# bupt-ai-cz/HIAST

Measured on AMD Instinct MI355X. Metric: self-training images/sec (fwd+bwd+pseudo-label) at 1024x512, higher is better.
Workload: dtype fp16

## Files before the change

### hiast_amd/_lib.py

```python
import ctypes
import os

import torch

_HERE = os.path.dirname(os.path.abspath(__file__))
LIB_PATH = os.environ.get("HIAST_LIB") or os.path.join(_HERE, "csrc", "libhiast_hip.so")

c_int, c_i64, c_f32, c_sz, c_vp = (ctypes.c_int, ctypes.c_int64, ctypes.c_float, ctypes.c_size_t,
                                   ctypes.c_void_p)

SIGNATURES = {
    "hiast_version": (c_int, []),
    "hiast_error_string": (ctypes.c_char_p, [c_int]),
    "hiast_upsample_bilinear_ac_fwd": (c_int, [c_vp, c_vp] + [c_int] * 6 + [c_vp]),
    "hiast_upsample_bilinear_ac_bwd": (c_int, [c_vp, c_vp] + [c_int] * 6 + [c_vp]),
    "hiast_plabel_pass1_workspace_bytes": (c_sz, [c_int]),
    "hiast_plabel_pass1": (c_int, [c_vp] + [c_int] * 6 + [c_vp, c_vp, c_vp, c_vp, c_sz, c_vp]),
    "hiast_plabel_pass2": (c_int, [c_vp, c_vp, c_vp, c_int, c_int, c_i64, c_vp, c_vp, c_vp, c_vp]),
    "hiast_plabel_strided_hist_workspace_bytes": (c_sz, [c_i64, c_int]),
    "hiast_plabel_strided_hist": (c_int, [c_vp, c_vp, c_i64, c_int, c_int, c_vp, c_vp, c_vp, c_vp, c_sz, c_vp]),
    "hiast_tta_fused": (c_int, [c_vp] * 6 + [c_int] * 5 + [c_vp, c_vp, c_vp]),
    "hiast_dinput_fwd": (c_int, [c_vp, c_int, c_vp] + [c_int] * 6 + [c_vp]),
    "hiast_dinput_bwd": (c_int, [c_vp, c_int, c_vp, c_vp, c_vp] + [c_int] * 6 + [c_vp]),
    "hiast_st_loss_workspace_bytes": (c_sz, [c_int] * 6),
    "hiast_st_loss_fwd": (c_int, [c_vp, c_vp, c_vp] + [c_int] * 8 + [c_vp, c_vp, c_sz, c_vp]),
    "hiast_st_loss_bwd": (c_int, [c_vp, c_vp, c_vp] + [c_int] * 8 + [c_vp, c_vp, c_vp, c_vp, c_sz, c_vp]),
    "hiast_aspp_wpack_bytes": (c_sz, [c_int, c_int]),
    "hiast_aspp_workspace_bytes": (c_sz, [c_int] * 5),
    "hiast_aspp_pack_weights": (c_int, [c_vp] * 8 + [c_int, c_int, c_vp, c_vp]),
    "hiast_aspp_fwd": (c_int, [c_vp, c_vp, c_vp] + [c_int] * 5 + [c_vp, c_vp, c_sz, c_vp]),
    "hiast_aspp_bwd_data": (c_int, [c_vp, c_vp, c_vp] + [c_int] * 5 + [c_vp, c_vp]),
    "hiast_aspp_bwd_weight": (c_int, [c_vp] * 7 + [c_int] * 5 + [c_vp, c_vp, c_sz, c_vp]),
    "hiast_aspp2_np": (c_int, [c_int]),
    "hiast_aspp2_workspace_bytes": (c_sz, [c_int] * 6),
    "hiast_aspp2_pack_weights": (c_int, [c_vp] * 8 + [c_int, c_int, c_vp, c_vp, c_vp, c_vp]),
    "hiast_aspp2_fwd": (c_int, [c_vp, c_int, c_vp, c_vp, c_vp] + [c_int] * 5 + [c_vp, c_vp, c_sz, c_vp]),
    "hiast_aspp2_bwd": (c_int, [c_vp] * 9 + [c_int] * 5 + [c_vp, c_int, c_vp, c_sz, c_vp]),
    "hiast_bn_workspace_bytes": (c_sz, [c_int, c_int]),
    "hiast_bn_stats": (c_int, [c_vp, c_int, c_int, c_i64, c_int, c_vp, c_vp]),
    "hiast_bn_act_apply": (c_int, [c_vp] * 8 + [c_int, ctypes.c_double, c_f32, c_f32, c_int, c_vp, c_vp,
                                   c_int, c_int, c_i64, c_int, c_vp]),
    "hiast_bn_act_bwd_stats": (c_int, [c_vp] * 5 + [c_int, c_int, c_int, c_i64, c_int, c_vp, c_vp]),
    "hiast_bn_act_bwd_apply": (c_int, [c_vp] * 7 + [c_int, ctypes.c_double, c_int, c_vp, c_vp, c_vp, c_vp,
                                       c_int, c_int, c_i64, c_int, c_vp]),
    "hiast_bn_act_nhwc_infer": (c_int, [c_vp] * 6 + [c_f32, c_int, c_i64, c_int, c_int, c_vp]),
    "hiast_igemm_bn_act": (c_int, [c_vp] * 6 + [c_f32, c_vp, c_int, c_vp] + [c_int] * 10 + [c_vp, c_int, c_vp, c_int, c_vp]),
    "hiast_igemm_set_cosched": (c_int, [c_int]),
    "hiast_igemm_set_half": (c_int, [c_int]),
    "hiast_device_cus": (c_int, []),
    "hiast_set_reserve_cus": (c_int, [c_int]),
    "hiast_get_reserve_cus": (c_int, []),
    "hiast_stream_create_reserved": (c_int, [c_vp, c_int]),
    "hiast_stream_destroy": (c_int, [c_vp]),
    "hiast_igemm_stats_rows": (c_int, [c_i64, c_int, c_int, c_int, c_int]),
    "hiast_igemm_dgrad_bn_stats": (c_int, [c_vp, c_vp, c_vp] + [c_int] * 7 + [c_vp] * 6 + [c_int, c_int, c_vp]),
    "hiast_xconv_dgrad_gated_bn_stats_rows": (c_int, [c_i64, c_int, c_int]),
    "hiast_xconv_dgrad_gated_bn_stats": (c_int, [c_vp] * 10 + [c_i64, c_int, c_int, c_int, c_vp]),
    "hiast_igemm_dgrad_s2": (c_int, [c_vp, c_vp, c_vp] + [c_int] * 6 + [c_vp]),
    "hiast_igemm_dgrad_bn_stats_rows": (c_int, [c_i64, c_int, c_int, c_int]),
    "hiast_bn_nhwc_stats_from_partial": (c_int, [c_vp, c_int, c_int, c_vp, c_vp]),
    "hiast_conv_wgrad_workspace_bytes": (c_sz, [c_int] * 6),
    "hiast_conv_wgrad_nhwc": (c_int, [c_vp, c_vp, c_vp] + [c_int] * 9 + [c_vp, c_sz, c_vp]),
    "hiast_conv_wgrad_group_workspace_bytes": (c_sz, [c_vp, c_int]),
    "hiast_conv_wgrad_group_nhwc": (c_int, [c_vp, c_int, c_int, c_vp, c_sz, c_vp]),
    "hiast_conv_wgrad_small_workspace_bytes": (c_sz, [c_int] * 6),
    "hiast_conv_wgrad_small_nhwc": (c_int, [c_vp, c_vp, c_vp] + [c_int] * 9 + [c_vp, c_sz, c_vp]),
    "hiast_pack_conv_weight": (c_int, [c_vp, c_int, c_int, c_int, c_int, c_int, c_vp, c_vp, c_vp]),
    "hiast_bn_nhwc_workspace_bytes": (c_sz, [c_int]),
    "hiast_bn_nhwc_stats": (c_int, [c_vp, c_i64, c_int, c_vp, c_vp, c_sz, c_int, c_vp]),
    "hiast_bn_nhwc_apply": (c_int, [c_vp] * 8 + [ctypes.c_double, c_f32, c_f32, c_int, c_vp, c_vp, c_i64, c_int, c_vp,
                                    c_int, c_vp]),
    "hiast_bn_nhwc_apply_partial": (c_int, [c_vp] * 8 + [c_int, ctypes.c_double, c_f32, c_f32, c_int, c_vp, c_vp, c_i64,
                                            c_int, c_vp, c_int, c_vp]),
    "hiast_bn_nhwc_bwd_stats": (c_int, [c_vp] * 7 + [c_int, c_i64, c_int, c_vp, c_vp, c_sz, c_int, c_vp]),
    "hiast_bn_nhwc_bwd_apply": (c_int, [c_vp] * 8 + [ctypes.c_double, c_int, c_vp, c_vp, c_vp, c_vp, c_i64, c_int, c_int,
                                        c_vp]),
    "hiast_pack_conv_weight_multi": (c_int, [c_vp, c_vp, c_vp, c_int, c_int, c_vp]),
    "hiast_split_planes": (c_int, [c_vp, c_vp, c_i64, c_int, c_int, c_vp]),
    "hiast_stem_tail": (c_int, [c_vp, c_int, c_vp, c_vp, c_vp, c_vp, c_f32, c_vp, c_int, c_int, c_int, c_int, c_int, c_vp]),
    "hiast_stem_eval": (c_int, [c_vp] * 6 + [c_f32, c_vp, c_int, c_int, c_int, c_int, c_vp]),
    "hiast_stem_train_blocks": (c_int, [c_int] * 3),
    "hiast_stem_train_fwd": (c_int, [c_vp, c_vp, c_vp, c_vp, c_int, c_int, c_int, c_int, c_vp]),
    "hiast_stem_wgrad_workspace_bytes": (c_sz, [c_int] * 3),
    "hiast_stem_wgrad": (c_int, [c_vp, c_vp, c_vp, c_int, c_int, c_int, c_int, c_vp, c_sz, c_vp]),
    "hiast_ema_update": (c_int, [c_vp, c_vp, c_vp, c_int, c_f32, c_f32, c_vp]),
    "hiast_normalize_u8": (c_int, [c_vp, c_vp, c_int, c_i64, c_vp, c_vp, c_vp]),
    "hiast_maxpool3x3s2_nhwc_fwd": (c_int, [c_vp, c_vp, c_vp, c_int, c_int, c_int, c_int, c_int, c_vp]),
    "hiast_maxpool3x3s2_nhwc_bwd": (c_int, [c_vp, c_vp, c_vp, c_int, c_int, c_int, c_int, c_int, c_vp]),
    "hiast_multi_copy": (c_int, [c_vp, c_int, c_vp]),
    "hiast_aug_geometry_u8": (c_int, [c_vp] * 6 + [c_int] * 4 + [c_vp]),
    "hiast_aug_hist_u8": (c_int, [c_vp] * 5 + [c_int, c_i64, c_vp]),
    "hiast_aug_colour_u8": (c_int, [c_vp] * 5 + [c_int, c_i64, c_vp]),
    "hiast_adam_prepare": (c_int, [c_vp, c_vp, c_vp, c_vp]),
    "hiast_adam_step": (c_int, [c_vp, c_vp, c_vp, c_int, ctypes.c_double, ctypes.c_double, c_f32, c_f32, c_vp, c_vp]),
    "hiast_confusion_hist": (c_int, [c_vp, c_vp, c_i64, c_int, c_vp, c_vp, c_vp, c_vp]),
}



class WgradJob(ctypes.Structure):
    _fields_ = [("dy", c_vp), ("x", c_vp), ("dw", c_vp)] + [(n, ctypes.c_int32) for n in
                                                             ("B", "H", "W", "Cin", "Cout", "taps", "stride", "dil")]


NBINS = 15361
PROB_FX_SHIFT = 30
IGNORE = 255

_lib = None


class HiastLibraryError(RuntimeError):
    pass


def load():
    global _lib
    if _lib is not None:
        return _lib
    if not os.path.exists(LIB_PATH):
        raise HiastLibraryError(
            "libhiast_hip.so is not built (%s). Build it with `python -c 'import __graft_entry__ as g; "
            "g.build()'` or `make -C hiast_amd/csrc`; there is no fallback path." % LIB_PATH)
    lib = ctypes.CDLL(LIB_PATH)
    for name, (res, args) in SIGNATURES.items():
        try:
            fn = getattr(lib, name)
        except AttributeError as e:
            raise HiastLibraryError("libhiast_hip.so does not export %s" % name) from e
        fn.restype = res
        fn.argtypes = args
    if lib.hiast_version() != 6:
        raise HiastLibraryError("libhiast_hip.so ABI version mismatch")
    _lib = lib
    return lib


# ... 17 lines not shown
```

### hiast_amd/csrc/igemm.hip

```cpp
#include "igemm_kernel.h"

namespace hiast {

template <int PL>
__device__ __forceinline__ size_t ig_wp_elem(int n, int t, int k, int taps, int KO)
{
    const size_t row = ((size_t)n * taps + t) * PL * KO;
    return PL == 2 ? row + (size_t)(k >> 5) * 64 + (k & 31) : row + k;
}

template <int PL, bool F16 = false>
__global__ __launch_bounds__(256) void pack_conv_weight_kernel(const float* __restrict__ w,
                                                               unsigned short* __restrict__ wp,
                                                               unsigned short* __restrict__ wpt, int N, int K, int taps,
                                                               int mode)
{
    const long long idx = (long long)blockIdx.x * 256 + threadIdx.x;
    if (idx >= (long long)N * taps * K) return;
    const int k = (int)(idx % K);
    const int t = (int)((idx / K) % taps);
    const int n = (int)(idx / ((long long)K * taps));
    const float v = w[((size_t)n * K + k) * taps + t];
    unsigned short h, l = 0;
    if (F16) h = H16<true>::enc(v);
// ... 104 lines not shown
        const int c = (int)((i * 8) - m * C);
        const float4 a = reinterpret_cast<const float4*>(x)[2 * i], b = reinterpret_cast<const float4*>(x)[2 * i + 1];
        const float v[8] = {a.x, a.y, a.z, a.w, b.x, b.y, b.z, b.w};
        unsigned ph[4], pl_[4];
#pragma unroll
        for (int q = 0; q < 4; ++q) {
            unsigned short h0, l0, h1, l1;
            ig_split(v[2 * q], h0, l0);
            ig_split(v[2 * q + 1], h1, l1);
            ph[q] = (unsigned)h0 | ((unsigned)h1 << 16);
            pl_[q] = (unsigned)l0 | ((unsigned)l1 << 16);
        }
        unsigned short* dst = p + ig_elem<2>((size_t)m, c, C);
        *reinterpret_cast<uint4*>(dst) = make_uint4(ph[0], ph[1], ph[2], ph[3]);
        *reinterpret_cast<uint4*>(dst + 32) = make_uint4(pl_[0], pl_[1], pl_[2], pl_[3]);
    }
}

__global__ __launch_bounds__(256) void from_planes_kernel(const unsigned short* __restrict__ p, float* __restrict__ x,
                                                          long long M, int C)
{
    const long long total8 = M * C / 8;
    for (long long i = (long long)blockIdx.x * 256 + threadIdx.x; i < total8; i += (long long)gridDim.x * 256) {
        const long long m = (i * 8) / C;
        const int c = (int)((i * 8) - m * C);
        const unsigned short* src = p + ig_elem<2>((size_t)m, c, C);
        const uint4 h = *reinterpret_cast<const uint4*>(src), l = *reinterpret_cast<const uint4*>(src + 32);
        const unsigned wh[4] = {h.x, h.y, h.z, h.w}, wl[4] = {l.x, l.y, l.z, l.w};
        float v[8];
#pragma unroll
        for (int q = 0; q < 4; ++q) {
            v[2 * q] = __uint_as_float(wh[q] << 16) + __uint_as_float(wl[q] << 16);
            v[2 * q + 1] = __uint_as_float(wh[q] & 0xFFFF0000u) + __uint_as_float(wl[q] & 0xFFFF0000u);
        }
        reinterpret_cast<float4*>(x)[2 * i] = make_float4(v[0], v[1], v[2], v[3]);
        reinterpret_cast<float4*>(x)[2 * i + 1] = make_float4(v[4], v[5], v[6], v[7]);
    }
}

}

const IgEnv& hiast_ig_env()
{
    static const IgEnv env = [] {
        IgEnv e;
        const char* v = getenv("HIAST_IGEMM_HALF");
        e.half = v ? (atoi(v) != 0) : -1;
        v = getenv("HIAST_IGEMM_BN");
        const int bn = v ? atoi(v) : 0;
        e.bn = (bn == 64 || bn == 128 || bn == 256) ? bn : 0;
        e.ragged_off = getenv("HIAST_IGEMM_RAGGED") != nullptr;
        v = getenv("HIAST_IGEMM_COSCHED");
        e.cosched0 = v && atoi(v) != 0;
        return e;
    }();
    return env;
}
static thread_local int ig_cosched_tls = -1, ig_half_tls = -1;
int hiast_ig_cosched_tls_get() { return ig_cosched_tls; }
int hiast_ig_half_tls_get() { return ig_half_tls; }
extern "C" int hiast_igemm_set_half(int v)
{
    const int prev = ig_half_tls;
    ig_half_tls = v < 0 ? -1 : (v != 0);
    return prev;
}
extern "C" int hiast_igemm_set_cosched(int on)
{
    const int prev = ig_cosched_tls;
    ig_cosched_tls = on < 0 ? -1 : (on != 0);
    return prev;
}

int hiast_xconv_ok(int64_t M, int K, int N, int planes, int taps, int out_f32, int has_bn, int has_res, int relu,
                   int has_gate, int gate_mask, int has_stats);
int hiast_xconv_stats_rows(int64_t M, int N);
int hiast_xconv_launch(const void* x, const void* wp, const float* gamma, const float* beta, const float* mean,
                       const float* var, float eps, const void* res, int relu, void* y, int64_t M, int K, int N,
                       float* stats, const void* res_gate, int f16, hipStream_t st);
int hiast_xconv2_ok(int64_t M, int K, int N, int planes, int taps, int out_f32, int has_bn, int has_res, int relu,
                    int has_gate, int has_stats);
int hiast_xconv2_launch(const void* x, const void* wp, const float* gamma, const float* beta, const float* mean,
                        const float* var, float eps, const void* res, int relu, void* y, int64_t M, int N, hipStream_t st);
int hiast_igemm_launch_f16(const void* x, const void* wp, const float* gamma, const float* beta, const float* mean,
                           const float* var, float eps, const void* res, int relu, void* y, int64_t M, int K, int N, int taps,
                           hiast::IGeo geo, float* stats, const void* res_gate, int gate_mask, hipStream_t st, int stats_mode,
                           int out_f32, int stats_rows);

static int igemm_launch_mode(const void* x, const void* wp, const float* gamma, const float* beta, const float* mean,
                             const float* var, float eps, const void* res, int relu, void* y, int64_t M, int K, int N,
                             int taps, int H, int W, int stride, int dil, int fmt, int out_f32, hipStream_t st,
                             float* stats, const void* res_gate, int gate_mask, int stats_mode, int stats_rows)
{
    if (!hiast_fmt_ok(fmt)) return HIAST_E_RANGE;
    const int planes = hiast_fmt_planes(fmt), f16 = fmt == HIAST_FMT_FP16;
    if (stats_mode == 2) {
        if (!stats || !res || !mean || !var || planes != 1 || out_f32 || relu || res_gate || N % 8) return HIAST_E_RANGE;
    } else {
        if (stats && (planes != 1 || out_f32 || res || relu)) return HIAST_E_RANGE;
        if ((stats || res_gate) && mean) return HIAST_E_RANGE;
    }
    if (res_gate && (planes != 1 || !res || relu || out_f32 || (!gate_mask && (((uintptr_t)res_gate) & 15)))) return HIAST_E_RANGE;
    if (!x || !wp || !y || (mean && !var)) return HIAST_E_ARG;
    if (M <= 0 || K <= 0 || N <= 0) return HIAST_E_ARG;
    if ((planes != 1 && planes != 2) || (taps != 1 && taps != 9)) return HIAST_E_RANGE;
    if ((K * planes) % 64 != 0 || N % 64 != 0 || M > (1ll << 31) - 512) return HIAST_E_RANGE;
    if (out_f32 && res) return HIAST_E_RANGE;
    if ((((uintptr_t)x) | ((uintptr_t)wp) | ((uintptr_t)y) | ((uintptr_t)res)) & 15) return HIAST_E_RANGE;
    hiast::IGeo geo = {0, 0, 0, 0, 1, 1};
    size_t in_pix = (size_t)M;
    if (taps != 1 && stride == -2) {
        if (H <= 0 || W <= 0 || dil != 1 || planes != 1 || out_f32) return HIAST_E_ARG;
        const int Hs = (H - 1) / 2 + 1, Ws = (W - 1) / 2 + 1;
        if (M % ((int64_t)H * W) != 0) return HIAST_E_ARG;
        geo = {Hs, Ws, H, W, -2, 1};
        in_pix = (size_t)(M / ((int64_t)H * W)) * Hs * Ws;
    } else if (taps != 1) {
        if (H <= 0 || W <= 0 || stride <= 0 || dil <= 0) return HIAST_E_ARG;
        const int Ho = (H - 1) / stride + 1, Wo = (W - 1) / stride + 1;
        if (M % ((int64_t)Ho * Wo) != 0) return HIAST_E_ARG;
        geo = {H, W, Ho, Wo, stride, dil};
        in_pix = (size_t)(M / ((int64_t)Ho * Wo)) * H * W;
    }
    if (in_pix * planes * K * 2 >= (1ull << 31) || (size_t)N * taps * planes * K * 2 >= (1ull << 31)) return HIAST_E_RANGE;
    if (stats_mode != 2 &&
        hiast_xconv_ok(M, K, N, planes, taps, out_f32, mean != nullptr, res != nullptr, relu, res_gate != nullptr, gate_mask,
                       stats != nullptr)) {
        if (stats && stats_rows != hiast_xconv_stats_rows(M, N)) return HIAST_E_ARG;
        return hiast_xconv_launch(x, wp, gamma, beta, mean, var, eps, res, relu, y, M, K, N, stats, res_gate, f16, st);
    }
    if (stats_mode == 0 && !f16 &&
        hiast_xconv2_ok(M, K, N, planes, taps, out_f32, mean != nullptr, res != nullptr, relu, res_gate != nullptr, stats != nullptr))
        return hiast_xconv2_launch(x, wp, gamma, beta, mean, var, eps, res, relu, y, M, N, st);
    if (f16)
        return hiast_igemm_launch_f16(x, wp, gamma, beta, mean, var, eps, res, relu, y, M, K, N, taps, geo, stats, res_gate,
                                      gate_mask, st, stats_mode, out_f32, stats_rows);
    if (planes == 2) {
        if (out_f32) return launch_igemm_t<2, true>(x, wp, gamma, beta, mean, var, eps, res, relu, y, M, K, N, taps, geo, stats, res_gate, gate_mask, st, stats_mode, stats_rows);
        return launch_igemm_t<2, false>(x, wp, gamma, beta, mean, var, eps, res, relu, y, M, K, N, taps, geo, stats, res_gate, gate_mask, st, stats_mode, stats_rows);
    }
    if (out_f32) return launch_igemm_t<1, true>(x, wp, gamma, beta, mean, var, eps, res, relu, y, M, K, N, taps, geo, stats, res_gate, gate_mask, st, stats_mode, stats_rows);
    return launch_igemm_t<1, false>(x, wp, gamma, beta, mean, var, eps, res, relu, y, M, K, N, taps, geo, stats, res_gate, gate_mask, st, stats_mode, stats_rows);
}

int hiast_igemm_launch(const void* x, const void* wp, const float* gamma, const float* beta, const float* mean,
                       const float* var, float eps, const void* res, int relu, void* y, int64_t M, int K, int N,
                       int taps, int H, int W, int stride, int dil, int fmt, int out_f32, hipStream_t st,
                       float* stats, const void* res_gate, int gate_mask, int stats_rows)
{
    return igemm_launch_mode(x, wp, gamma, beta, mean, var, eps, res, relu, y, M, K, N, taps, H, W, stride, dil, fmt,
                             out_f32, st, stats, res_gate, gate_mask, stats ? 1 : 0, stats_rows);
}

extern "C" int hiast_igemm_dgrad_bn_stats(const void* dy, const void* wpt, void* da, int B, int H, int W, int Cin, int Cout,
                                          int taps, int dil, const void* bn_x, const float* gamma, const float* beta,
                                          const float* save_mean, const float* save_invstd, float* partial, int partial_rows,
                                          int fmt, hiast_stream_t stream)
{
    if (fmt != HIAST_FMT_BF16 && fmt != HIAST_FMT_FP16) return HIAST_E_RANGE;
    if (B <= 0 || H <= 0 || W <= 0) return HIAST_E_ARG;
    if (!bn_x || !save_mean || !save_invstd || !partial) return HIAST_E_ARG;
    if ((((uintptr_t)save_mean) | ((uintptr_t)save_invstd) | ((uintptr_t)gamma) | ((uintptr_t)beta)) & 15) return HIAST_E_RANGE;
    return igemm_launch_mode(dy, wpt, gamma, beta, save_mean, save_invstd, 0.0f, bn_x, 0, da, (int64_t)B * H * W, Cin, Cout,
                             taps, H, W, 1, dil, fmt, 0, (hipStream_t)stream, partial, nullptr, 0, 2, partial_rows);
}

extern "C" int hiast_igemm_dgrad_s2(const void* dy, const void* wpt, void* dx, int B, int H, int W, int Cin, int Cout, int fmt,
                                    hiast_stream_t stream)
{
    if (fmt != HIAST_FMT_BF16 && fmt != HIAST_FMT_FP16) return HIAST_E_RANGE;
    if (B <= 0 || H <= 0 || W <= 0) return HIAST_E_ARG;
    return igemm_launch_mode(dy, wpt, nullptr, nullptr, nullptr, nullptr, 0.0f, nullptr, 0, dx, (int64_t)B * H * W, Cout, Cin, 9,
                             H, W, -2, 1, fmt, 0, (hipStream_t)stream, nullptr, nullptr, 0, 0, 0);
}

extern "C" int hiast_igemm_dgrad_bn_stats_rows(int64_t M, int Cin, int Cout, int taps)
{
    if (M <= 0) return 0;
    const int bm = ig_block_rows(M, Cin, Cout, taps, 0);
    return (int)((M + bm - 1) / bm);
}

extern "C" int hiast_igemm_bn_act(const void* x, const void* wp, const float* gamma, const float* beta,
                                  const float* mean, const float* var, float eps, const void* res, int relu, void* y,
                                  int B, int H, int W, int Cin, int Cout, int taps, int stride, int dil, int fmt,
                                  int out_f32, float* stats, int stats_rows, const void* res_gate, int gate_mask,
                                  hiast_stream_t stream)
{
    if (B <= 0 || H <= 0 || W <= 0) return HIAST_E_ARG;
    if (taps == 1 && stride != 1) return HIAST_E_RANGE;
    const int Ho = taps == 1 ? H : (H - 1) / stride + 1, Wo = taps == 1 ? W : (W - 1) / stride + 1;
    return hiast_igemm_launch(x, wp, gamma, beta, mean, var, eps, res, relu, y, (int64_t)B * Ho * Wo, Cin, Cout, taps, H,
                              W, stride, dil, fmt, out_f32, (hipStream_t)stream, stats, res_gate, gate_mask, stats_rows);
}

#ifdef IG_STAMP
namespace hiast {
__global__ void ig_stamp_copy_kernel(unsigned* dst)
{
    for (int i = blockIdx.x * blockDim.x + threadIdx.x; i < 1024 * 8 * 8 + 32 * 64; i += gridDim.x * blockDim.x) dst[i] = ig_stamp_buf[i];
}
}
extern "C" int hiast_igemm_debug_stamps(unsigned* dst_device)
{
    hipLaunchKernelGGL(hiast::ig_stamp_copy_kernel, dim3(64), dim3(256), 0, 0, dst_device);
    return (int)hipDeviceSynchronize();
}
#endif

extern "C" int hiast_igemm_stats_rows(int64_t M, int Cin, int Cout, int taps, int fmt)
{
    const int planes = hiast_fmt_planes(fmt);
    if (M <= 0 || Cin <= 0 || Cout <= 0) return 0;
    if (hiast_xconv_ok(M, Cin, Cout, planes, taps, 0, 0, 0, 0, 0, 0, 1)) return hiast_xconv_stats_rows(M, Cout);
    const int bm = ig_block_rows(M, Cin, Cout, taps, 0);
    return (int)((M + bm - 1) / bm);
}

extern "C" int hiast_pack_conv_weight(const float* w, int N, int K, int taps, int fmt, int transpose, void* wp,
                                      void* wpt, hiast_stream_t stream)
{
    if (!w || !wp) return HIAST_E_ARG;
    if (N <= 0 || K <= 0 || taps <= 0) return HIAST_E_ARG;
    const int planes = fmt;
    if (!hiast_fmt_ok(fmt) || transpose < 0 || transpose > 2) return HIAST_E_RANGE;
    if (transpose == 2 && !wpt) return HIAST_E_ARG;
    const long long total = (long long)N * K * taps;
    if (N % 64 == 0 && K % 64 == 0 && taps <= 9 && !((((uintptr_t)wp) | ((uintptr_t)wpt)) & 15)) {
        const dim3 tg((unsigned)((N / 64) * (K / 64)));
        const size_t lds_bytes = (size_t)32 * taps * hiast::PK_PITCH * sizeof(unsigned short);
        if (planes == HIAST_FMT_SPLIT_BF16)
            hipLaunchKernelGGL(hiast::pack_conv_weight_tiled_kernel<2>, tg, dim3(256), lds_bytes, (hipStream_t)stream, w,
                               (unsigned short*)wp, (unsigned short*)wpt, N, K, taps, transpose);
        else if (planes == HIAST_FMT_FP16)
            hipLaunchKernelGGL((hiast::pack_conv_weight_tiled_kernel<1, true>), tg, dim3(256), lds_bytes, (hipStream_t)stream, w,
                               (unsigned short*)wp, (unsigned short*)wpt, N, K, taps, transpose);
        else
            hipLaunchKernelGGL(hiast::pack_conv_weight_tiled_kernel<1>, tg, dim3(256), lds_bytes, (hipStream_t)stream, w,
                               (unsigned short*)wp, (unsigned short*)wpt, N, K, taps, transpose);
        HIAST_CHECK_LAUNCH();
        return 0;
    }
    const dim3 grid((unsigned)((total + 255) / 256));
    if (planes == HIAST_FMT_SPLIT_BF16)
        hipLaunchKernelGGL(hiast::pack_conv_weight_kernel<2>, grid, dim3(256), 0, (hipStream_t)stream, w,
                           (unsigned short*)wp, (unsigned short*)wpt, N, K, taps, transpose);
    else if (planes == HIAST_FMT_FP16)
        hipLaunchKernelGGL((hiast::pack_conv_weight_kernel<1, true>), grid, dim3(256), 0, (hipStream_t)stream, w,
                           (unsigned short*)wp, (unsigned short*)wpt, N, K, taps, transpose);
    else
        hipLaunchKernelGGL(hiast::pack_conv_weight_kernel<1>, grid, dim3(256), 0, (hipStream_t)stream, w,
                           (unsigned short*)wp, (unsigned short*)wpt, N, K, taps, transpose);
    HIAST_CHECK_LAUNCH();
    return 0;
}

namespace hiast {

template <int INK, int PL, bool F16 = false>
__global__ __launch_bounds__(256) void stem_tail_kernel(const void* __restrict__ xv, const float* __restrict__ gamma,
                                                        const float* __restrict__ beta, const float* __restrict__ mean,
                                                        const float* __restrict__ var, float eps,
                                                        unsigned short* __restrict__ out, int B, int H, int W, int C, int Ho,
                                                        int Wo)
{
    const int G = C >> 3;
    const long long total = (long long)B * Ho * Wo * G;
    const long long stride = (long long)gridDim.x * 256;
    long long i = (long long)blockIdx.x * 256 + threadIdx.x;
    if (i >= total) return;
    const int cg = (int)(i % G);
    float sc[8], sh[8];
#pragma unroll
    for (int k = 0; k < 8; ++k) {
        const int c = cg * 8 + k;
        const float invstd = 1.0f / sqrtf(var[c] + eps);
        sc[k] = (gamma ? gamma[c] : 1.0f) * invstd;
        sh[k] = fmaf(-mean[c], sc[k], beta ? beta[c] : 0.0f);
    }
    for (; i < total; i += stride) {
        const long long pix = i / G;
        const int xo = (int)(pix % Wo);
        const int yo = (int)((pix / Wo) % Ho);
        const int b = (int)(pix / ((long long)Wo * Ho));
        float m[8];
#pragma unroll
        for (int k = 0; k < 8; ++k) m[k] = -INFINITY;
#pragma unroll
        for (int dy = 0; dy < 3; ++dy) {
            const int yy = 2 * yo - 1 + dy;
            if (yy < 0 || yy >= H) continue;
#pragma unroll
            for (int dx = 0; dx < 3; ++dx) {
                const int xx = 2 * xo - 1 + dx;
                if (xx < 0 || xx >= W) continue;
                const size_t off = (((size_t)b * H + yy) * W + xx) * C + cg * 8;
                float v[8];
// ... 115 lines not shown
```

### include/hiast_hip.h

```cpp
#ifndef HIAST_HIP_H
#define HIAST_HIP_H

#include <stddef.h>
#include <stdint.h>

#ifdef __cplusplus
extern "C" {
#endif

#define HIAST_ABI_VERSION 6

#define HIAST_E_ARG   (-1)
#define HIAST_E_RANGE (-2)
#define HIAST_E_WS    (-3)

#define HIAST_NBINS 15361
#define HIAST_PROB_FX_SHIFT 30
#define HIAST_MAX_CLASSES 32
#define HIAST_FMT_BF16 1
#define HIAST_FMT_SPLIT_BF16 2
#define HIAST_FMT_FP16 3
#define HIAST_IGNORE 255

typedef void* hiast_stream_t;
// ... 15 lines not shown
size_t hiast_plabel_pass1_workspace_bytes(int C);
int hiast_plabel_pass1(const float* logits_lr, int B, int C, int h, int w, int H, int W,
                       float* maxprob, uint8_t* argmax, uint32_t* hist, void* workspace,
                       size_t workspace_bytes, hiast_stream_t stream);

int hiast_plabel_pass2(const float* maxprob, const uint8_t* argmax, const float* thr_up,
                       int B, int C, int64_t HW, uint8_t* plbl, int64_t* count,
                       uint64_t* sumprob_fx, hiast_stream_t stream);

size_t hiast_plabel_strided_hist_workspace_bytes(int64_t N, int C);
int hiast_plabel_strided_hist(const float* maxprob, const uint8_t* argmax, int64_t N, int C, int interval,
                              const int64_t* rank_offset, int64_t* class_total, uint32_t* hist,
                              void* workspace, size_t workspace_bytes, hiast_stream_t stream);

#define HIAST_TTA_MAX_SCALES 8
int hiast_tta_fused(const float* const* z, const float* const* zf, const int* hs, const int* ws, const int* Hs,
                    const int* Ws, int n_scales, int B, int C, int H, int W, float* probsum, uint8_t* label,
                    hiast_stream_t stream);

size_t hiast_st_loss_workspace_bytes(int B, int C, int h, int w, int H, int W);
int hiast_st_loss_fwd(const float* logits_lr, const float* teacher_lr, const void* plbl,
                      int plbl_is_i64, int B, int C, int h, int w, int H, int W, int region,
                      double* sums, void* workspace, size_t workspace_bytes,
                      hiast_stream_t stream);
int hiast_st_loss_bwd(const float* logits_lr, const float* teacher_lr, const void* plbl,
                      int plbl_is_i64, int B, int C, int h, int w, int H, int W, int region,
                      const double* sums, const float* coef, float* dlogits_lr,
                      void* workspace, size_t workspace_bytes, hiast_stream_t stream);

size_t hiast_aspp_wpack_bytes(int Cin, int Cout);
size_t hiast_aspp_workspace_bytes(int B, int Cin, int h, int w, int Cout);
int hiast_aspp_pack_weights(const float* w0, const float* w1, const float* w2, const float* w3,
                            const float* b0, const float* b1, const float* b2, const float* b3,
                            int Cin, int Cout, float* wpack, hiast_stream_t stream);
int hiast_aspp_fwd(const float* x, const float* wpack, float* y, int B, int Cin, int h, int w,
                   int Cout, const int* dil, void* workspace, size_t workspace_bytes,
                   hiast_stream_t stream);
int hiast_aspp_bwd_data(const float* dy, const float* wpack, float* dx, int B, int Cin, int h,
                        int w, int Cout, const int* dil, hiast_stream_t stream);
int hiast_aspp_bwd_weight(const float* x, const float* dy, float* dw0, float* dw1, float* dw2,
                          float* dw3, float* db, int B, int Cin, int h, int w, int Cout,
                          const int* dil, void* workspace, size_t workspace_bytes,
                          hiast_stream_t stream);

int hiast_aspp2_np(int Cout);
size_t hiast_aspp2_workspace_bytes(int B, int Cin, int h, int w, int Cout, int backward);
int hiast_aspp2_pack_weights(const float* w0, const float* w1, const float* w2, const float* w3,
                             const float* b0, const float* b1, const float* b2, const float* b3, int Cin,
                             int Cout, float* wt, float* wd, float* bias, hiast_stream_t stream);
int hiast_aspp2_fwd(const void* x_nhwc, int dtype, const void* wt, const float* bias, float* y, int B, int Cin,
                    int h, int w, int Cout, const int* dil, void* workspace, size_t workspace_bytes,
                    hiast_stream_t stream);
int hiast_aspp2_bwd(const void* x_nhwc, const float* dy, const void* wd, void* dx_nhwc, float* dw0, float* dw1,
                    float* dw2, float* dw3, float* db, int B, int Cin, int h, int w, int Cout, const int* dil,
                    int fmt ,
                    void* workspace, size_t workspace_bytes, hiast_stream_t stream);

size_t hiast_bn_workspace_bytes(int B, int C);
int hiast_bn_stats(const void* x, int B, int C, int64_t HW, int dtype, double* part, hiast_stream_t stream);
int hiast_bn_act_apply(const void* x, const void* res, void* y, const float* gamma, const float* beta,
                       float* running_mean, float* running_var, const double* part, int npart, double count,
                       float momentum, float eps, int relu, float* save_mean, float* save_invstd, int B, int C,
                       int64_t HW, int dtype, hiast_stream_t stream);
int hiast_bn_act_bwd_stats(const void* dy, const void* y, const void* x, const float* save_mean,
                           const float* save_invstd, int relu, int B, int C, int64_t HW, int dtype,
                           double* part, hiast_stream_t stream);
int hiast_bn_act_bwd_apply(const void* dy, const void* y, const void* x, const float* gamma,
                           const float* save_mean, const float* save_invstd, const double* part, int npart,
                           double count, int relu, void* dx, void* dres, float* dgamma, float* dbeta, int B,
                           int C, int64_t HW, int dtype, hiast_stream_t stream);

int hiast_bn_act_nhwc_infer(const void* x, void* y, const float* gamma, const float* beta, const float* mean,
                            const float* var, float eps, int relu, int64_t M, int C, int dtype,
                            hiast_stream_t stream);

int hiast_igemm_bn_act(const void* x, const void* wp, const float* gamma, const float* beta, const float* mean,
                       const float* var, float eps, const void* res, int relu, void* y, int B, int H, int W, int Cin,
                       int Cout, int taps, int stride, int dil, int fmt , int out_f32, float* stats,
                       int stats_rows ,
                       const void* res_gate, int gate_mask, hiast_stream_t stream);
int hiast_igemm_set_cosched(int on);
int hiast_igemm_set_half(int v);
int hiast_igemm_stats_rows(int64_t M, int Cin, int Cout, int taps, int fmt);
int hiast_igemm_dgrad_bn_stats(const void* dy, const void* wpt, void* da, int B, int H, int W, int Cin, int Cout, int taps,
                               int dil, const void* bn_x, const float* gamma, const float* beta, const float* save_mean,
                               const float* save_invstd, float* partial, int partial_rows ,
                               int fmt , hiast_stream_t stream);
int hiast_igemm_dgrad_bn_stats_rows(int64_t M, int Cin, int Cout, int taps);
int hiast_igemm_dgrad_s2(const void* dy, const void* wpt, void* dx, int B, int H, int W, int Cin, int Cout, int fmt,
                         hiast_stream_t stream);
int hiast_xconv_dgrad_gated_bn_stats_rows(int64_t M, int K, int N);
int hiast_xconv_dgrad_gated_bn_stats(const void* dy, const void* wpt, const void* res, const void* res_gate, const void* bn_x,
                                     const void* bn_mask, const float* save_mean, const float* save_invstd, void* dx,
                                     float* partial, int64_t M, int K, int N, int fmt, hiast_stream_t stream);
int hiast_pack_conv_weight(const float* w, int N, int K, int taps, int fmt, int transpose, void* wp, void* wpt,
                           hiast_stream_t stream);
int hiast_split_planes(float* x, void* planes, int64_t M, int C, int inverse, hiast_stream_t stream);
int hiast_stem_tail(const void* x, int dtype , const float* gamma, const float* beta,
                    const float* mean, const float* var, float eps, void* out, int fmt , int B, int H,
                    int W, int C, hiast_stream_t stream);
int hiast_stem_eval(const float* x, const float* w, const float* gamma, const float* beta, const float* mean, const float* var,
                    float eps, void* out, int fmt, int B, int H, int W, hiast_stream_t stream);

int hiast_stem_train_blocks(int B, int H, int W);
int hiast_stem_train_fwd(const float* x, const float* w, void* y, float* partial, int fmt, int B, int H, int W,
                         hiast_stream_t stream);
size_t hiast_stem_wgrad_workspace_bytes(int B, int H, int W);
int hiast_stem_wgrad(const float* x, const void* dy, float* dw, int fmt, int B, int H, int W, void* workspace,
                     size_t workspace_bytes, hiast_stream_t stream);
typedef struct { const float* w; void* wp; void* wpt; int32_t N, K, taps, planes , mode, pad; } hiast_pack_rec;
int hiast_pack_conv_weight_multi(const hiast_pack_rec* table, const int32_t* chunk_tensor, const int64_t* chunk_start,
                                 int n_chunks, int max_taps, hiast_stream_t stream);

size_t hiast_conv_wgrad_workspace_bytes(int B, int Ho, int Wo, int Cin, int Cout, int taps);
int hiast_conv_wgrad_nhwc(const void* dy, const void* x, float* dw, int B, int H, int W, int Cin, int Cout, int taps,
                          int stride, int dil, int fmt ,
                          void* workspace, size_t workspace_bytes, hiast_stream_t stream);

typedef struct { const void* dy; const void* x; float* dw; int32_t B, H, W, Cin, Cout, taps, stride, dil; } hiast_wgrad_job;
size_t hiast_conv_wgrad_group_workspace_bytes(const hiast_wgrad_job* jobs, int njobs);
int hiast_conv_wgrad_group_nhwc(const hiast_wgrad_job* jobs, int njobs, int fmt, void* workspace, size_t workspace_bytes,
                                hiast_stream_t stream);

size_t hiast_conv_wgrad_small_workspace_bytes(int B, int H, int W, int Cin, int Cout, int taps);
int hiast_conv_wgrad_small_nhwc(const void* dy, const void* x, float* dw, int B, int H, int W, int Cin, int Cout, int taps,
                                int stride, int dil, int fmt, void* workspace, size_t workspace_bytes, hiast_stream_t stream);

size_t hiast_bn_nhwc_workspace_bytes(int C);
int hiast_bn_nhwc_stats(const void* x, int64_t M, int C, double* sums, void* workspace, size_t workspace_bytes, int fmt,
                        hiast_stream_t stream);
int hiast_bn_nhwc_stats_from_partial(const float* partial, int nblk, int C, double* sums, hiast_stream_t stream);
int hiast_bn_nhwc_apply_partial(const void* x, const void* res, void* y, const float* gamma, const float* beta,
                                float* running_mean, float* running_var, const float* partial, int nblk, double count,
                                float momentum, float eps, int relu, float* save_mean, float* save_invstd, int64_t M,
                                int C, void* mask, int fmt, hiast_stream_t stream);
int hiast_bn_nhwc_apply(const void* x, const void* res, void* y, const float* gamma, const float* beta,
                        float* running_mean, float* running_var, const double* sums, double count, float momentum,
                        float eps, int relu, float* save_mean, float* save_invstd, int64_t M, int C, void* mask, int fmt,
                        hiast_stream_t stream);
int hiast_bn_nhwc_bwd_stats(const void* dy, const void* y, const void* x, const float* gamma, const float* beta,
                            const float* save_mean, const float* save_invstd, int relu, int64_t M, int C, double* sums,
                            void* workspace, size_t workspace_bytes, int fmt, hiast_stream_t stream);
int hiast_bn_nhwc_bwd_apply(const void* dy, const void* y, const void* x, const float* gamma, const float* beta,
                            const float* save_mean, const float* save_invstd, const double* sums, double count, int relu,
                            void* dx, void* dres, float* dgamma, float* dbeta, int64_t M, int C, int fmt,
                            hiast_stream_t stream);

typedef struct { float* ema; const float* p; int64_t n; } hiast_ema_rec;
int hiast_ema_update(const hiast_ema_rec* table, const int32_t* chunk_tensor,
                     const int64_t* chunk_start, int n_chunks, float gamma,
                     float one_minus_gamma, hiast_stream_t stream);

int hiast_maxpool3x3s2_nhwc_fwd(const void* x, void* y, uint8_t* idx, int B, int H, int W, int C,
                                int fmt , hiast_stream_t stream);
int hiast_maxpool3x3s2_nhwc_bwd(const void* dy, const uint8_t* idx, void* dx, int B, int H, int W, int C, int fmt,
                                hiast_stream_t stream);

int hiast_normalize_u8(const uint8_t* img, float* out, int B, int64_t HW, const float* mean, const float* std,
                       hiast_stream_t stream);

#define HIAST_AUG_REC_WORDS 20
#define HIAST_AUG_MAX_OPS 8
#define HIAST_AUG_OPS_WORDS (4 + 2 * HIAST_AUG_MAX_OPS)
#define HIAST_AUG_OP_LUT 1
#define HIAST_AUG_OP_GRAY 2
#define HIAST_AUG_OP_EQUALIZE 3
// ... 31 lines not shown
```

Before: 142.8.

## Add persistent weight-stationary 1x1 conv kernel for K=512, N=2048 GEMMs

Adds a specialised persistent GEMM kernel for 1x1 convolutions with 512 input and 2048 output channels. Each block keeps its 256-column weight slice in registers, streams 32-row input panels through a 3-stage LDS ring filled by buffer-to-LDS DMA, and fuses BN, residual, gated-residual and batch-statistics epilogues. The generic igemm dispatch and the stats-row sizing route matching shapes to it. In exchange it adds heavy register pressure, a rigid shape gate and new launch variants, and an environment switch can turn it off.

Result: no change. 142.9 (median of 2 runs) (+0.0%).

```diff
diff --git a/hiast_amd/_lib.py b/hiast_amd/_lib.py
--- a/hiast_amd/_lib.py
+++ b/hiast_amd/_lib.py
@@ -53,6 +53,7 @@
     "hiast_stream_create_reserved": (c_int, [c_vp, c_int]),
     "hiast_stream_destroy": (c_int, [c_vp]),
     "hiast_igemm_stats_rows": (c_int, [c_i64, c_int, c_int, c_int, c_int]),
+    "hiast_xconv512_ok": (c_int, [c_i64] + [c_int] * 11),
     "hiast_igemm_dgrad_bn_stats": (c_int, [c_vp, c_vp, c_vp] + [c_int] * 7 + [c_vp] * 6 + [c_int, c_int, c_vp]),
     "hiast_xconv_dgrad_gated_bn_stats_rows": (c_int, [c_i64, c_int, c_int]),
     "hiast_xconv_dgrad_gated_bn_stats": (c_int, [c_vp] * 10 + [c_i64, c_int, c_int, c_int, c_vp]),
diff --git a/hiast_amd/csrc/igemm.hip b/hiast_amd/csrc/igemm.hip
--- a/hiast_amd/csrc/igemm.hip
+++ b/hiast_amd/csrc/igemm.hip
@@ -210,6 +210,10 @@
                     int has_gate, int has_stats);
 int hiast_xconv2_launch(const void* x, const void* wp, const float* gamma, const float* beta, const float* mean,
                         const float* var, float eps, const void* res, int relu, void* y, int64_t M, int N, hipStream_t st);
+int hiast_xconv512_stats_rows(int64_t M, int N);
+int hiast_xconv512_launch(const void* x, const void* wp, const float* gamma, const float* beta, const float* mean,
+                          const float* var, float eps, const void* res, int relu, void* y, int64_t M, int N, float* stats,
+                          const void* res_gate, int f16, hipStream_t st);
 int hiast_igemm_launch_f16(const void* x, const void* wp, const float* gamma, const float* beta, const float* mean,
                            const float* var, float eps, const void* res, int relu, void* y, int64_t M, int K, int N, int taps,
                            hiast::IGeo geo, float* stats, const void* res_gate, int gate_mask, hipStream_t st, int stats_mode,
@@ -260,6 +264,12 @@
     if (stats_mode == 0 && !f16 &&
         hiast_xconv2_ok(M, K, N, planes, taps, out_f32, mean != nullptr, res != nullptr, relu, res_gate != nullptr, stats != nullptr))
         return hiast_xconv2_launch(x, wp, gamma, beta, mean, var, eps, res, relu, y, M, N, st);
+    if (stats_mode != 2 &&
+        hiast_xconv512_ok(M, K, N, planes, taps, out_f32, mean != nullptr, res != nullptr, relu, res_gate != nullptr, gate_mask,
+                          stats != nullptr)) {
+        if (stats && stats_rows != hiast_xconv512_stats_rows(M, N)) return HIAST_E_ARG;
+        return hiast_xconv512_launch(x, wp, gamma, beta, mean, var, eps, res, relu, y, M, N, stats, res_gate, f16, st);
+    }
     if (f16)
         return hiast_igemm_launch_f16(x, wp, gamma, beta, mean, var, eps, res, relu, y, M, K, N, taps, geo, stats, res_gate,
                                       gate_mask, st, stats_mode, out_f32, stats_rows);
@@ -341,6 +351,7 @@
     const int planes = hiast_fmt_planes(fmt);
     if (M <= 0 || Cin <= 0 || Cout <= 0) return 0;
     if (hiast_xconv_ok(M, Cin, Cout, planes, taps, 0, 0, 0, 0, 0, 0, 1)) return hiast_xconv_stats_rows(M, Cout);
+    if (hiast_xconv512_ok(M, Cin, Cout, planes, taps, 0, 0, 0, 0, 0, 0, 1)) return hiast_xconv512_stats_rows(M, Cout);
     const int bm = ig_block_rows(M, Cin, Cout, taps, 0);
     return (int)((M + bm - 1) / bm);
 }
diff --git a/hiast_amd/csrc/xconv512.hip b/hiast_amd/csrc/xconv512.hip
--- /dev/null
+++ b/hiast_amd/csrc/xconv512.hip
@@ -0,0 +1,297 @@
+#include <hip/hip_bf16.h>
+#include <stdlib.h>
+
+#include <type_traits>
+
+#include "common.h"
+
+namespace hiast {
+
+typedef __attribute__((ext_vector_type(8))) __bf16 x5_bf16x8;
+typedef __attribute__((address_space(3))) void* x5_lds_ptr;
+
+constexpr int X5_PANEL = 32;
+constexpr int X5_STAGES = 3;
+constexpr int X5_COLS = 256;
+constexpr int X5_K = 512;
+constexpr int X5_ROWB = X5_K * 2;
+constexpr int X5_STAGE = X5_PANEL * X5_ROWB;
+
+__device__ __forceinline__ void x5_dma16(__amdgpu_buffer_rsrc_t rs, unsigned char* lds, int voff, int soff)
+{
+    __builtin_amdgcn_raw_ptr_buffer_load_lds(rs, (x5_lds_ptr)lds, 16, voff, soff, 0, 0);
+}
+
+__device__ __forceinline__ int x5_lds_off(int row, int chunk) { return row * 128 + ((chunk ^ ((row >> 1) & 7)) << 4); }
+
+template <int OFF>
+__device__ __forceinline__ x5_bf16x8 x5_lds_read(unsigned addr)
+{
+    x5_bf16x8 v;
+    asm volatile("ds_read_b128 %0, %1 offset:%2" : "=v"(v) : "v"(addr), "i"(OFF));
+    return v;
+}
+__device__ __forceinline__ void x5_lds_wait(x5_bf16x8& a, x5_bf16x8& b, x5_bf16x8& c, x5_bf16x8& d)
+{
+    asm volatile("s_waitcnt lgkmcnt(0)" : "+v"(a), "+v"(b), "+v"(c), "+v"(d));
+}
+
+template <bool BN, bool RES, bool RELU, bool GATE, bool STATS, bool F16>
+__global__ __launch_bounds__(512) void xconv512_kernel(const unsigned short* __restrict__ X,
+                                                       const unsigned short* __restrict__ Wp,
+                                                       const float* __restrict__ gamma, const float* __restrict__ beta,
+                                                       const float* __restrict__ mean, const float* __restrict__ var,
+                                                       float eps, const unsigned short* __restrict__ R,
+                                                       const unsigned char* __restrict__ Rg,
+                                                       unsigned short* __restrict__ Y, int M, int N,
+                                                       float* __restrict__ stats)
+{
+    static_assert(!GATE || (RES && !RELU && !BN), "gated residual: data-gradient launches only");
+    static_assert(!STATS || (!BN && !RES && !RELU), "statistics epilogue: the plain GEMM only");
+    using HT = H16<F16>;
+    constexpr int KS = X5_K / 64;
+    __shared__ __attribute__((aligned(1024))) unsigned char smem[X5_STAGES * X5_STAGE];
+    __shared__ float s_sc[BN ? X5_COLS : 1], s_sh[BN ? X5_COLS : 1];
+
+    const int tid = threadIdx.x, lane = tid & 63;
+    const int wave = __builtin_amdgcn_readfirstlane(tid >> 6);
+    const int g = lane >> 4, px = lane & 15;
+    const int NG = N / X5_COLS;
+    const int xcd = blockIdx.x & 7, slot = blockIdx.x >> 3;
+    const int cg = slot % NG;
+    const int nstream = (int)gridDim.x / NG;
+    const int stream = (slot / NG) * 8 + xcd;
+    const int n0 = cg * X5_COLS + wave * 32;
+    const int npanel = (M + X5_PANEL - 1) / X5_PANEL;
+
+    x5_bf16x8 w0[2][KS], w1[2][KS];
+#pragma unroll
+    for (int b = 0; b < 2; ++b) {
+        const unsigned short* wrow = Wp + (size_t)(n0 + (px >> 2) * 8 + b * 4 + (px & 3)) * X5_K + g * 8;
+#pragma unroll
+        for (int s = 0; s < KS; ++s) {
+            w0[b][s] = *reinterpret_cast<const x5_bf16x8*>(wrow + s * 64);
+            w1[b][s] = *reinterpret_cast<const x5_bf16x8*>(wrow + s * 64 + 32);
+        }
+    }
+#pragma unroll
+    for (int b = 0; b < 2; ++b)
+#pragma unroll
+        for (int s = 0; s < KS; ++s) asm volatile("" : "+v"(w0[b][s]), "+v"(w1[b][s]));
+    if (BN) {
+        for (int c = tid; c < X5_COLS; c += 512) {
+            const int n = cg * X5_COLS + c;
+            const float sc = (gamma ? gamma[n] : 1.0f) * (1.0f / sqrtf(var[n] + eps));
+            s_sc[c] = sc;
+            s_sh[c] = fmaf(-mean[n], sc, beta ? beta[n] : 0.0f);
+        }
+        __syncthreads();
+    }
+
+    constexpr int OOB = (int)0x80000000;
+    const __amdgpu_buffer_rsrc_t xrs = __builtin_amdgcn_make_buffer_rsrc((void*)X, 0, (int)((size_t)M * X5_ROWB), 0x00020000);
+    const int rgrp = wave & 3, j0 = (wave >> 2) * 4;
+    const int drow = rgrp * 8 + (lane >> 3);
+    const int dchunk = ((lane & 7) ^ ((drow >> 1) & 7)) * 16;
+    auto issue = [&](int p, int st) {
+        const int m = p * X5_PANEL + drow;
+        const int voff = (p < npanel && m < M) ? (int)((size_t)m * X5_ROWB) + dchunk : OOB;
+        unsigned char* base = smem + st * X5_STAGE + rgrp * 1024;
+#pragma unroll
+        for (int j = 0; j < 4; ++j) x5_dma16(xrs, base + (j0 + j) * (X5_PANEL * 128), voff, (j0 + j) * 128);
+    };
+    const unsigned lds_base = (unsigned)(size_t)smem;
+
+    constexpr int NRES = RES ? (GATE ? 4 : 2) : 0;
+    auto row_off = [&](int m) { return (size_t)(m < M ? m : 0) * N + n0 + g * 8; };
+    uint4 rr[2][2];
+    unsigned rgate[2][2];
+    auto load_res = [&](int p, int buf) {
+#pragma unroll
+        for (int a = 0; a < 2; ++a) {
+            const int m = (p < npanel ? p : 0) * X5_PANEL + a * 16 + px;
+            rr[buf][a] = h_load16_once(R + row_off(m));
+            if (GATE) rgate[buf][a] = Rg[(size_t)(m < M ? m : 0) * (N >> 3) + ((n0 + g * 8) >> 3)];
+        }
+    };
+    float st1[STATS ? 8 : 1], st2[STATS ? 8 : 1];
+#pragma unroll
+    for (int q = 0; q < (STATS ? 8 : 1); ++q) { st1[q] = 0.f; st2[q] = 0.f; }
+
+    const int pfirst = stream, pstep = nstream;
+    auto valid = [&](int p) { return p < npanel; };
+    issue(valid(pfirst) ? pfirst : npanel, 0);
+    issue(valid(pfirst + pstep) ? pfirst + pstep : npanel, 1);
+    if (RES) load_res(valid(pfirst) ? pfirst : 0, 0);
+
+    auto panel = [&](int p, int it, auto cur_tag) {
+        constexpr int CUR = decltype(cur_tag)::value;
+        const int st = it % X5_STAGES;
+        if (it == 0) asm volatile("s_waitcnt vmcnt(%0)\n\ts_barrier" ::"n"(4 + NRES) : "memory");
+        else asm volatile("s_waitcnt vmcnt(%0)\n\ts_barrier" ::"n"(4 + 2 + NRES) : "memory");
+        if (RES) load_res(valid(p + pstep) ? p + pstep : 0, CUR ^ 1);
+        issue(valid(p + 2 * pstep) ? p + 2 * pstep : npanel, (it + 2) % X5_STAGES);
+
+        h_f32x4 acc[2][2];
+#pragma unroll
+        for (int a = 0; a < 2; ++a)
+#pragma unroll
+            for (int b = 0; b < 2; ++b) acc[a][b] = (h_f32x4){0.f, 0.f, 0.f, 0.f};
+        const unsigned fa = lds_base + (unsigned)(st * X5_STAGE + x5_lds_off(px, g));
+        const unsigned fb = fa ^ 64u;
+        x5_bf16x8 x0[2][2], x1[2][2];
+#define X5_READ(S, RG)                                                                                              \
+        x0[RG][0] = x5_lds_read<(S) * 4096>(fa);        x1[RG][0] = x5_lds_read<(S) * 4096>(fb);                    \
+        x0[RG][1] = x5_lds_read<(S) * 4096 + 2048>(fa); x1[RG][1] = x5_lds_read<(S) * 4096 + 2048>(fb);
+#define X5_STEP(S, RG)                                                                                              \
+        x5_lds_wait(x0[RG][0], x1[RG][0], x0[RG][1], x1[RG][1]);                                                    \
+        if ((S) + 1 < 8) { X5_READ(((S) + 1) & 7, (RG) ^ 1) }                                                        \
+        _Pragma("unroll") for (int a = 0; a < 2; ++a)                                                               \
+            _Pragma("unroll") for (int b = 0; b < 2; ++b) {                \
+                acc[a][b] = HT::mfma16(w0[b][S], x0[RG][a], acc[a][b]);                                             \
+                acc[a][b] = HT::mfma16(w1[b][S], x1[RG][a], acc[a][b]);                                             \
+            }
+        X5_READ(0, 0)
+        X5_STEP(0, 0) X5_STEP(1, 1) X5_STEP(2, 0) X5_STEP(3, 1) X5_STEP(4, 0) X5_STEP(5, 1) X5_STEP(6, 0) X5_STEP(7, 1)
+#undef X5_STEP
+#undef X5_READ
+        static_assert(KS == 8, "eight slabs");
+        float sc[8], sh[8];
+        if (BN) {
+            const int c0 = wave * 32 + g * 8;
+            const float4 s0 = *reinterpret_cast<const float4*>(&s_sc[c0]), s1 = *reinterpret_cast<const float4*>(&s_sc[c0 + 4]);
+            const float4 t0 = *reinterpret_cast<const float4*>(&s_sh[c0]), t1 = *reinterpret_cast<const float4*>(&s_sh[c0 + 4]);
+            sc[0] = s0.x; sc[1] = s0.y; sc[2] = s0.z; sc[3] = s0.w; sc[4] = s1.x; sc[5] = s1.y; sc[6] = s1.z; sc[7] = s1.w;
+            sh[0] = t0.x; sh[1] = t0.y; sh[2] = t0.z; sh[3] = t0.w; sh[4] = t1.x; sh[5] = t1.y; sh[6] = t1.z; sh[7] = t1.w;
+        }
+#pragma unroll
+        for (int a = 0; a < 2; ++a) {
+            const int m = p * X5_PANEL + a * 16 + px;
+            const bool ok = m < M;
+            float o[8];
+#pragma unroll
+            for (int b = 0; b < 2; ++b)
+#pragma unroll
+                for (int r = 0; r < 4; ++r)
+                    o[b * 4 + r] = BN ? fmaf(acc[a][b][r], sc[b * 4 + r], sh[b * 4 + r]) : acc[a][b][r];
+            if (RES) {
+                const uint4 v = rr[CUR][a];
+                const unsigned w4[4] = {v.x, v.y, v.z, v.w};
+                const unsigned gate = GATE ? rgate[CUR][a] : 0xFFu;
+#pragma unroll
+                for (int q = 0; q < 4; ++q) {
+                    float r0 = HT::lo(w4[q]), r1 = HT::hi(w4[q]);
+                    if (GATE) {
+                        r0 = ((gate >> (2 * q)) & 1u) ? r0 : 0.f;
+                        r1 = ((gate >> (2 * q + 1)) & 1u) ? r1 : 0.f;
+                    }
+                    o[2 * q] += r0;
+                    o[2 * q + 1] += r1;
+                }
+            }
+            if (RELU) {
+#pragma unroll
+                for (int q = 0; q < 8; ++q) o[q] = o[q] > 0.f ? o[q] : 0.f;
+            }
+            unsigned pk[4];
+#pragma unroll
+            for (int q = 0; q < 4; ++q) pk[q] = HT::pack(o[2 * q], o[2 * q + 1]);
+            if (STATS && ok) {
+#pragma unroll
+                for (int q = 0; q < 4; ++q) {
+                    const float v0 = HT::lo(pk[q]), v1 = HT::hi(pk[q]);
+                    st1[2 * q] += v0; st2[2 * q] = fmaf(v0, v0, st2[2 * q]);
+                    st1[2 * q + 1] += v1; st2[2 * q + 1] = fmaf(v1, v1, st2[2 * q + 1]);
+                }
+            }
+            if (ok) h_store16_out(Y + row_off(m), pk[0], pk[1], pk[2], pk[3]);
+        }
+    };
+    int it = 0, p = pfirst;
+    for (; valid(p + pstep); p += 2 * pstep, it += 2) {
+        panel(p, it, std::integral_constant<int, 0>());
+        panel(p + pstep, it + 1, std::integral_constant<int, 1>());
+    }
+    if (valid(p)) panel(p, it, std::integral_constant<int, 0>());
+    if (STATS) {
+#pragma unroll
+        for (int q = 0; q < 8; ++q) {
+#pragma unroll
+            for (int o = 1; o < 16; o <<= 1) {
+                st1[q] += __shfl_xor(st1[q], o, 64);
+                st2[q] += __shfl_xor(st2[q], o, 64);
+            }
+        }
+        if (px == 0) {
+            float* d = stats + ((size_t)stream * N + n0 + g * 8) * 2;
+#pragma unroll
+            for (int q = 0; q < 8; ++q) {
+                d[2 * q] = st1[q];
+                d[2 * q + 1] = st2[q];
+            }
+        }
+    }
+}
+
+static int x5_blocks(int64_t M, int N)
+{
+    const int NG = N / X5_COLS;
+    const long long npanel = (M + X5_PANEL - 1) / X5_PANEL;
+    static const int env_cus = [] { const char* e = getenv("HIAST_XCONV_CUS"); const int v = e ? atoi(e) : 0; return v >= 8 && v <= 256 ? v : 0; }();
+    const int cus = env_cus ? env_cus : hiast_grid_cus();
+    long long streams = cus / NG / 8 * 8;
+    if (streams < 8) streams = 8;
+    if (streams > npanel) streams = (npanel + 7) / 8 * 8;
+    return (int)(streams * NG);
+}
+
+}
+
+extern "C" int hiast_xconv512_ok(int64_t M, int K, int N, int planes, int taps, int out_f32, int has_bn, int has_res, int relu,
+                                 int has_gate, int gate_mask, int has_stats)
+{
+    const char* env = getenv("HIAST_XCONV512");
+    if ((env && atoi(env) == 0) || planes != 1 || taps != 1 || out_f32) return 0;
+    if (K != hiast::X5_K || N != 2048) return 0;
+    if (M < 4096 || M > (1ll << 31) / hiast::X5_ROWB - 64) return 0;
+    if (has_stats) return !(has_bn || has_res || relu || has_gate);
+    if (has_gate) return gate_mask && has_res && !relu && !has_bn;
+    if (has_bn) return has_res && relu;
+    return !relu;
+}
+
+int hiast_xconv512_stats_rows(int64_t M, int N)
+{
+    return hiast::x5_blocks(M, N) / (N / hiast::X5_COLS);
+}
+
+int hiast_xconv512_launch(const void* x, const void* wp, const float* gamma, const float* beta, const float* mean,
+                          const float* var, float eps, const void* res, int relu, void* y, int64_t M, int N, float* stats,
+                          const void* res_gate, int f16, hipStream_t st)
+{
+    using namespace hiast;
+    const dim3 grid((unsigned)x5_blocks(M, N));
+#define X5L(BNF, RESF, RELUF, GATEF, STATSF)                                                                          \
+    do {                                                                                                              \
+        if (f16)                                                                                                      \
+            hipLaunchKernelGGL((xconv512_kernel<BNF, RESF, RELUF, GATEF, STATSF, true>), grid, dim3(512), 0, st,       \
+                               (const unsigned short*)x, (const unsigned short*)wp, gamma, beta, mean, var, eps,      \
+                               (const unsigned short*)res, (const unsigned char*)res_gate, (unsigned short*)y, (int)M, N, \
+                               stats);                                                                                \
+        else                                                                                                          \
+            hipLaunchKernelGGL((xconv512_kernel<BNF, RESF, RELUF, GATEF, STATSF, false>), grid, dim3(512), 0, st,      \
+                               (const unsigned short*)x, (const unsigned short*)wp, gamma, beta, mean, var, eps,      \
+                               (const unsigned short*)res, (const unsigned char*)res_gate, (unsigned short*)y, (int)M, N, \
+                               stats);                                                                                \
+    } while (0)
+    const bool bn = mean != nullptr;
+    if (stats) { if (bn || res || relu || res_gate) return HIAST_E_RANGE; X5L(false, false, false, false, true); }
+    else if (res_gate) { if (bn || !res || relu) return HIAST_E_RANGE; X5L(false, true, false, true, false); }
+    else if (bn) { if (!res || !relu) return HIAST_E_RANGE; X5L(true, true, true, false, false); }
+    else if (relu) return HIAST_E_RANGE;
+    else if (res) X5L(false, true, false, false, false);
+    else X5L(false, false, false, false, false);
+#undef X5L
+    HIAST_CHECK_LAUNCH();
+    return 0;
+}
diff --git a/include/hiast_hip.h b/include/hiast_hip.h
--- a/include/hiast_hip.h
+++ b/include/hiast_hip.h
@@ -121,6 +121,8 @@
 int hiast_igemm_set_cosched(int on);
 int hiast_igemm_set_half(int v);
 int hiast_igemm_stats_rows(int64_t M, int Cin, int Cout, int taps, int fmt);
+int hiast_xconv512_ok(int64_t M, int K, int N, int planes, int taps, int out_f32, int has_bn, int has_res, int relu,
+                      int has_gate, int gate_mask, int has_stats);
 int hiast_igemm_dgrad_bn_stats(const void* dy, const void* wpt, void* da, int B, int H, int W, int Cin, int Cout, int taps,
                                int dil, const void* bn_x, const float* gamma, const float* beta, const float* save_mean,
                                const float* save_invstd, float* partial, int partial_rows ,
```
